# facebookresearch/ReAgent

Measured on NVIDIA H100. Metric: minibatch_td_updates_per_sec_b4096, higher is better.
Workload: dtype f32

## Files before the change

### reagent_b200/csrc/rb200_dqn_tc.cu

```cuda
#include <string.h>

#include <type_traits>

#include "rb200_dqn_tc_layout.cuh"
#include "rb200_wgmma.cuh"

namespace rb200 {

constexpr int kQR = 32;
constexpr int kQSub = 2;
constexpr int kQStages = 3;
constexpr int kQStageBytes = kQSub * (kQKC / 4) * kQFullLbo;
constexpr int kQLboB = 64 * 16 + 16;
constexpr int kQLoOff = 32 * 4;
constexpr int kQEpiThreads = 256;
constexpr int kQThreads = kQEpiThreads + 32;
constexpr int kQMaxTiles = 4;
constexpr int kQMaxSteps = 4 * kMaxLayers;
constexpr int kQMaxSmem = 232448;
static_assert(kQKC == 32, "a chunk is four K = 8 MMA steps");

enum { kStepHidden = 0, kStepLast = 1, kStepBwd = 2 };

struct QStep {
  uint32_t pack_off;
  int16_t N, K;
  int8_t layer, kind, net, in_buf, load_x, save, qdst, out_buf;
};

struct QDev {
  rb200_dqn_args_t a;
  rb200_net_ws_t ws;
  const unsigned char* pack;
  int nsteps, last_fwd_step;
  int buf_off[3];
  int q_off, ldq, lin_off, bar_off;
  int need_zero;
  QStep steps[kQMaxSteps];
};

struct PackJob {
  const float* W;
  int N, K;
  int ld;
  int transpose;
  uint32_t pack_off;
  int chunk0;
};
struct PackDev {
  PackJob jobs[3 * kMaxLayers];
  int njobs;
  unsigned char* pack;
};

constexpr int kPackParts = 4;

__global__ void __launch_bounds__(256) dqn_tc_pack_kernel(const PackDev p) {
  const int chunk = (int)blockIdx.x / kPackParts, part = (int)blockIdx.x % kPackParts;
  int j = 0;
  while (j + 1 < p.njobs && chunk >= p.jobs[j + 1].chunk0) ++j;
  const PackJob job = p.jobs[j];
  const int local = chunk - job.chunk0;
  const int kch = ceil_div(job.K, kQKC);
  const int t = local / kch, c = local - t * kch;
  const ChunkGeo g = chunk_geo(job.N, job.K, t, c);
  const int rows8 = (int)(g.lbo - 16) / 16, kl8 = g.ksteps * 8;
  float* img = reinterpret_cast<float*>(p.pack + job.pack_off + g.off);
  const int m0 = 128 * t, k0 = kQKC * c;
  const int total = rows8 * kl8;
  constexpr int U = 4;
  for (int base = (part * 256 + (int)threadIdx.x); base < total; base += kPackParts * 256 * U) {
    float v[U];
    int o[U];
#pragma unroll
    for (int u = 0; u < U; ++u) {
      const int idx = base + u * kPackParts * 256;
      int m, kk;
      if (job.transpose) { kk = idx / rows8; m = idx - kk * rows8; }
      else { m = idx / kl8; kk = idx - m * kl8; }
      v[u] = 0.f;
      o[u] = -1;
      if (idx < total) {
        o[u] = (kk >> 2) * (int)(g.lbo / 4) + m * 4 + (kk & 3);
        if (m0 + m < job.N && k0 + kk < job.K)
          v[u] = job.transpose ? __ldg(job.W + (size_t)(k0 + kk) * job.ld + m0 + m)
                               : __ldg(job.W + (size_t)(m0 + m) * job.ld + k0 + kk);
      }
    }
#pragma unroll
    for (int u = 0; u < U; ++u)
      if (o[u] >= 0) img[o[u]] = v[u];
  }
}

__device__ __noinline__ float act_fwd_slow(float x, int act) { return act_fwd(x, act); }
__device__ __noinline__ float act_bwd_slow(float y, int act) { return act_bwd_from_out(y, act); }

constexpr int kQCK = kQKC / 8;

template <int NK>
__device__ __forceinline__ void chunk_mma(float (&acc)[32], const uint32_t (&ah)[kQCK][4],
                                          const uint32_t (&al)[kQCK][4], uint32_t b0) {
  wgmma_fence();
#pragma unroll
  for (int kk = 0; kk < NK; ++kk) {
    const uint64_t bd = wgmma_desc(b0 + (uint32_t)(2 * kk) * kQLboB, kQLboB, 128);
    wgmma_rs_n64(acc, ah[kk], bd, 1u);
    wgmma_rs_n32(acc, al[kk], bd, 1u);
  }
  wgmma_commit();
}
template <int NK, typename F>
__device__ __forceinline__ void with_ksteps(int nk, F&& f) {
  if (nk == NK) f(std::integral_constant<int, NK>());
  else if constexpr (NK > 1) with_ksteps<NK - 1>(nk, f);
}

template <bool kWeighted>
__global__ void __launch_bounds__(kQThreads, 1)
dqn_td_tc_kernel(const Mlp q, const Mlp qt, const QDev p) {
  extern __shared__ __align__(128) unsigned char smem_raw[];
  const int tid = threadIdx.x, warp = tid >> 5, lane = tid & 31;
  const rb200_dqn_args_t& a = p.a;
  const int B = a.batch;
  const int row0 = blockIdx.x * kQR;
  const int L = q.n_layers;
  const int A = q.dims[L];

  if (p.need_zero) {
    unsigned nbytes;
    asm("mov.u32 %0, %%dynamic_smem_size;" : "=r"(nbytes));
    for (unsigned i = (unsigned)p.buf_off[0] + tid * 16u; i + 15u < nbytes; i += kQThreads * 16u)
      *reinterpret_cast<float4*>(smem_raw + i) = make_float4(0.f, 0.f, 0.f, 0.f);
  }
  __syncthreads();

  unsigned char* ring = smem_raw;
  float* qarr = reinterpret_cast<float*>(smem_raw + p.q_off);
  float* act_s = reinterpret_cast<float*>(smem_raw + p.lin_off);
  float* mask_s = act_s + kQR * A;
  float* scal_s = mask_s + kQR * A;
  uint64_t* full = reinterpret_cast<uint64_t*>(smem_raw + p.bar_off);
  uint64_t* sfree = full + kQStages;
  const int ldq = p.ldq;

  if (tid == 0) {
    for (int s = 0; s < kQStages; ++s) { mbar_init(full + s, 1); mbar_init(sfree + s, kQEpiThreads / 32); }
    asm volatile("fence.mbarrier_init.release.cluster;\n" ::: "memory");
  }
  __syncthreads();

  const int role = __shfl_sync(0xffffffffu, warp, 0);
  if (role == kQEpiThreads / 32) {
    const bool leader = elect_one();
    int stage = 0;
    uint32_t par = 1;
    for (int s = 0; s < p.nsteps; ++s) {
      const QStep st = p.steps[s];
      const int mt = ceil_div(st.N, 128), kch = ceil_div(st.K, kQKC);
      const uint32_t tile_stride = (uint32_t)(round_up8(st.K) / 4) * kQFullLbo;
      for (int t = 0; t < mt; ++t) {
        const int rows = st.N - 128 * t;
        const uint32_t lbo = (uint32_t)(round_up8(rows < 128 ? rows : 128) * 16 + 16);
        const uint32_t full_bytes = (kQKC / 4) * lbo;
        const int klast = st.K - kQKC * (kch - 1);
        const uint32_t last_bytes = (uint32_t)(round_up8(klast) / 4) * lbo;
        const unsigned char* src = p.pack + st.pack_off + (size_t)t * tile_stride;
        for (int c = 0; c < kch; c += kQSub) {
          const int nsub = kch - c < kQSub ? kch - c : kQSub;
          const uint32_t bytes = (uint32_t)(nsub - 1) * full_bytes + ((c + nsub == kch) ? last_bytes : full_bytes);
          mbar_wait(sfree + stage, par);
          if (leader) {
            mbar_expect_tx(full + stage, bytes);
            bulk_g2s(ring + stage * kQStageBytes, src, bytes, full + stage);
          }
          src += bytes;
          if (++stage == kQStages) { stage = 0; par ^= 1u; }
        }
      }
    }
  } else {
    const int wg = warp >> 2, w4 = warp & 3, g = lane >> 2, tq = lane & 3;
    int ss = 0;
    uint32_t spar = 0;

    constexpr int kXQ = 4;
    const int xS = q.dims[0];
    const int xnq = round_up8(xS) / 4;
    const bool x_in_regs = kQR * xnq <= kXQ * kQEpiThreads;
    float4 xr[kXQ];
    auto x_fetch_one = [&](const float* src, int idx) {
      const bool vec = ((xS & 3) == 0) && ((reinterpret_cast<uintptr_t>(src) & 15) == 0);
      const int r = idx / xnq, qd = idx - r * xnq;
      const int k = 4 * qd, row = row0 + r;
      float4 v = make_float4(0.f, 0.f, 0.f, 0.f);
      if (idx < kQR * xnq && row < B) {
        const float* sp = src + (size_t)row * xS;
        if (vec && k + 3 < xS) {
          asm volatile("ld.global.nc.v4.f32 {%0,%1,%2,%3}, [%4];\n"
                       : "=f"(v.x), "=f"(v.y), "=f"(v.z), "=f"(v.w)
                       : "l"(sp + k));
        } else {
          if (k < xS) v.x = sp[k];
          if (k + 1 < xS) v.y = sp[k + 1];
          if (k + 2 < xS) v.z = sp[k + 2];
          if (k + 3 < xS) v.w = sp[k + 3];
        }
      }
      return v;
    };
    auto x_store_one = [&](int idx, const float4 v) {
      if (idx >= kQR * xnq) return;
      float* base = reinterpret_cast<float*>(smem_raw + p.buf_off[0]);
      const int r = idx / xnq, qd = idx - r * xnq;
      float4 h, l;
      split4(v, h, l);
      const int o = qd * (kQLboB / 4) + r * 4;
      *reinterpret_cast<float4*>(base + o) = h;
      *reinterpret_cast<float4*>(base + o + kQLoOff) = l;
    };
    auto x_fetch = [&](const float* src) {
      if (!x_in_regs) return;
#pragma unroll
      for (int i = 0; i < kXQ; ++i) xr[i] = x_fetch_one(src, tid + i * kQEpiThreads);
    };
    auto x_store = [&](const float* src) {
      if (x_in_regs) {
#pragma unroll
        for (int i = 0; i < kXQ; ++i) x_store_one(tid + i * kQEpiThreads, xr[i]);
      } else {
        for (int idx = tid; idx < kQR * xnq; idx += kQEpiThreads) x_store_one(idx, x_fetch_one(src, idx));
      }
    };
    auto load_loss_inputs = [&]() {
      const float* mask = a.maxq ? a.possible_next_actions_mask : a.next_action;
      for (int idx = tid; idx < kQR * A; idx += kQEpiThreads) {
        const int r = idx / A;
        const bool in = row0 + r < B;
        const size_t g = (size_t)row0 * A + idx;
        act_s[idx] = in ? a.action[g] : 0.f;
        mask_s[idx] = (in && mask) ? mask[g] : 1.f;
      }
      if (tid < kQR) {
        const int row = row0 + tid;
        const bool in = row < B;
        scal_s[tid * 4 + 0] = in ? a.reward[row] : 0.f;
        scal_s[tid * 4 + 1] = in ? a.not_terminal[row] : 0.f;
        scal_s[tid * 4 + 2] = (in && a.discount_mode == RB200_DISCOUNT_POW) ? a.discount_src[row] : 0.f;
      }
    };
    auto step_tiles = [&](const QStep& st) {
      const Mlp& net = st.net ? qt : q;
      const int l = st.layer, N = st.N;
      const int mt = ceil_div(N, 128), kch = ceil_div(st.K, kQKC);
      float* obase = reinterpret_cast<float*>(smem_raw + p.buf_off[st.out_buf]);
      const uint32_t bbase = smem_u32(smem_raw + p.buf_off[st.in_buf]);
      for (int t = 0; t < mt; ++t) {
        const int rows = N - 128 * t;
        const int rows8 = round_up8(rows < 128 ? rows : 128);
        const uint32_t lbo = (uint32_t)(rows8 * 16 + 16);
        const bool live = 64 * wg < rows;
        const int m0 = 64 * wg + 16 * w4 + g;
        const bool ok0 = live && m0 < rows8, ok1 = live && m0 + 8 < rows8;
        float acc[32];
#pragma unroll
        for (int i = 0; i < 32; ++i) {
          acc[i] = 0.f;
          wgmma_fence_operand(acc[i]);
        }
        static_assert(kQSub == 2, "one fragment buffer per chunk of a ring stage");
        const int kfull = st.K / kQKC;
        const int nk_last = round_up8(st.K - kQKC * kfull) / 8;
        uint32_t ah[2][kQCK][4], al[2][kQCK][4];
        auto fetch = [&](uint32_t (&fh)[kQCK][4], uint32_t (&fl)[kQCK][4], int c, int nk) {
          if (c % 2 == 0) mbar_wait(full + ss, spar);
          float v[kQCK][4];
#pragma unroll
          for (int kk = 0; kk < kQCK; ++kk) {
            v[kk][0] = v[kk][1] = v[kk][2] = v[kk][3] = 0.f;
            const unsigned char* s0 = ring + ss * kQStageBytes + (uint32_t)((c % 2) * (kQKC / 4) + 2 * kk) * lbo + tq * 4;
            const unsigned char* s1 = s0 + lbo;
            if (kk < nk && ok0) { v[kk][0] = *reinterpret_cast<const float*>(s0 + m0 * 16); v[kk][2] = *reinterpret_cast<const float*>(s1 + m0 * 16); }
            if (kk < nk && ok1) { v[kk][1] = *reinterpret_cast<const float*>(s0 + (m0 + 8) * 16); v[kk][3] = *reinterpret_cast<const float*>(s1 + (m0 + 8) * 16); }
          }
          if (c % 2 == 1 || c + 1 == kch) {
            __syncwarp();
            if (lane == 0) mbar_arrive(sfree + ss);
            if (++ss == kQStages) { ss = 0; spar ^= 1u; }
          }
#pragma unroll
          for (int kk = 0; kk < kQCK; ++kk)
#pragma unroll
            for (int e = 0; e < 4; ++e) {
              float h, lo_;
              split1(v[kk][e], h, lo_);
              fh[kk][e] = __float_as_uint(h);
              fl[kk][e] = __float_as_uint(lo_);
              wgmma_fence_operand(fh[kk][e]);
              wgmma_fence_operand(fl[kk][e]);
            }
        };
        auto b_of = [&](int c) { return bbase + (uint32_t)(2 * kQCK * c) * kQLboB; };
        if (kfull > 0) fetch(ah[0], al[0], 0, kQCK);
        for (int c = 0; c < kfull; c += 2) {
          chunk_mma<kQCK>(acc, ah[0], al[0], b_of(c));
          if (c + 1 == kfull) break;
          wgmma_wait<1>();
          fetch(ah[1], al[1], c + 1, kQCK);
          chunk_mma<kQCK>(acc, ah[1], al[1], b_of(c + 1));
          if (c + 2 == kfull) break;
          wgmma_wait<1>();
          fetch(ah[0], al[0], c + 2, kQCK);
        }
        if (kfull < kch) {
          wgmma_wait<0>();
          fetch(ah[0], al[0], kfull, nk_last);
          with_ksteps<kQCK>(nk_last, [&](auto nk_c) {
            chunk_mma<decltype(nk_c)::value>(acc, ah[0], al[0], b_of(kfull));
          });
        }
        wgmma_wait<0>();
#pragma unroll
        for (int i = 0; i < 32; ++i) wgmma_fence_operand(acc[i]);
        if (!live) continue;

#pragma unroll
        for (int hh = 0; hh < 2; ++hh) {
          const int n = 128 * t + m0 + 8 * hh;
          const bool valid = n < N;
          float x[8];
#pragma unroll
          for (int i = 0; i < 4; ++i)
#pragma unroll
            for (int e = 0; e < 2; ++e) x[2 * i + e] = acc[4 * i + 2 * hh + e] + acc[4 * (i + 4) + 2 * hh + e];
          auto rowof = [&](int k) { return 8 * (k >> 1) + 2 * tq + (k & 1); };
          float* ob = obase + (n >> 2) * (kQLboB / 4) + (n & 3);
          bool to_operand, to_global;
          float* gdst = nullptr;
          if (st.kind == kStepBwd) {
            const int hact = q.act[l - 1];
            float hv[8];
            if (st.save) {
              const float* hs = p.ws.hidden[l - 1];
#pragma unroll
              for (int k = 0; k < 8; ++k) {
                const int row = row0 + rowof(k);
                hv[k] = (valid && row < B) ? hs[(size_t)row * N + n] : 0.f;
              }
            } else {
#pragma unroll
              for (int k = 0; k < 8; ++k) hv[k] = valid ? ob[rowof(k) * 4] + ob[rowof(k) * 4 + kQLoOff] : 0.f;
            }
            if (hact == RB200_ACT_RELU) {
#pragma unroll
              for (int k = 0; k < 8; ++k) x[k] = hv[k] > 0.f ? x[k] : 0.f;
            } else if (hact != RB200_ACT_LINEAR) {
#pragma unroll
              for (int k = 0; k < 8; ++k) x[k] = valid ? x[k] * act_bwd_slow(hv[k], hact) : 0.f;
            }
            to_operand = l - 1 >= 1;
            to_global = true;
            gdst = p.ws.dz[l - 1];
          } else {
            const float bias = valid ? __ldg(net.params + net.b_off[l] + n) : 0.f;
            const int act = net.act[l];
            if (act == RB200_ACT_RELU) {
#pragma unroll
              for (int k = 0; k < 8; ++k) x[k] = fmaxf(x[k] + bias, 0.f);
            } else if (act == RB200_ACT_LINEAR) {
#pragma unroll
              for (int k = 0; k < 8; ++k) x[k] += bias;
            } else {
#pragma unroll
              for (int k = 0; k < 8; ++k) x[k] = act_fwd_slow(x[k] + bias, act);
            }
            to_operand = st.kind != kStepLast;
            to_global = st.save != 0 && st.kind != kStepLast;
            gdst = to_global ? p.ws.hidden[l] : nullptr;
          }
          if (!valid) continue;
          if (st.kind == kStepLast) {
            float* qd = qarr + st.qdst * kQR * ldq + n;
#pragma unroll
            for (int k = 0; k < 8; ++k) qd[rowof(k) * ldq] = x[k];
            continue;
          }
          if (to_operand) {
#pragma unroll
            for (int k = 0; k < 8; ++k) {
              float h, lo_;
              split1(row0 + rowof(k) < B ? x[k] : 0.f, h, lo_);
              ob[rowof(k) * 4] = h;
              ob[rowof(k) * 4 + kQLoOff] = lo_;
            }
          }
          if (to_global) {
#pragma unroll
            for (int k = 0; k < 8; ++k) {
              const int row = row0 + rowof(k);
              if (row < B) gdst[(size_t)row * N + n] = x[k];
            }
          }
        }
      }
    };
    auto loss_stage = [&]() {
      const float* qa = qarr;
      const float* qb = qarr + kQR * ldq;
      const float* qc = qarr + 2 * kQR * ldq;
      const int r = tid >> 3, sub = tid & 7;
      const int row = row0 + r;
      const bool in = row < B;
      float best = 0.f, sel = 0.f, qsel = 0.f, bsum = 0.f;
      int bi = 0x7fffffff;
      for (int c = sub; c < A; c += 8) {
        const float pen = -1e9f * (1.f - mask_s[r * A + c]);
        const float vt = qb[r * ldq + c] + pen;
        const float key = a.double_q ? (qa[r * ldq + c] + pen) : vt;
        if (bi == 0x7fffffff || key > best) { best = key; bi = c; sel = vt; }
        const float aw = act_s[r * A + c];
        qsel += qc[r * ldq + c] * aw;
        if (a.reward_boost) bsum += aw * a.reward_boost[c];
      }
#pragma unroll
      for (int o = 1; o < 8; o <<= 1) {
        const float ob = __shfl_xor_sync(0xffffffffu, best, o);
        const float os = __shfl_xor_sync(0xffffffffu, sel, o);
        const int oi = __shfl_xor_sync(0xffffffffu, bi, o);
        qsel += __shfl_xor_sync(0xffffffffu, qsel, o);
        bsum += __shfl_xor_sync(0xffffffffu, bsum, o);
        if (oi != 0x7fffffff && (bi == 0x7fffffff || ob > best || (ob == best && oi < bi))) {
          best = ob; bi = oi; sel = os;
        }
      }
      float le = 0.f, g = 0.f;
      if (in) {
        const float rew = scal_s[r * 4 + 0] + bsum;
        const float disc = (a.discount_mode == RB200_DISCOUNT_POW)
                               ? powf(a.gamma, scal_s[r * 4 + 2]) : a.gamma;
        const float tgt = rew + disc * (sel * scal_s[r * 4 + 1]);
        const float d = qsel - tgt;
        const float invB = 1.f / (float)B;
        if (a.loss_kind == RB200_LOSS_HUBER) {
          const float ad = fabsf(d);
          le = ad < 1.f ? 0.5f * d * d : ad - 0.5f;
          g = (d < -1.f) ? -invB : (d > 1.f ? invB : invB * d);
        } else {
          le = d * d;
          g = 2.f * invB * d;
        }
        if (kWeighted) {
          const float w = a.sample_weight[row];
          le *= w;
          g *= w;
        }
        if (sub == 0) {
          if (a.td_target) a.td_target[row] = tgt;
          if (a.next_action_idx) a.next_action_idx[row] = bi;
          if (a.q_selected) a.q_selected[row] = qsel;
        }
      }
      const int A8 = round_up8(A);
      const int lact = q.act[L - 1];
      float* zb = reinterpret_cast<float*>(smem_raw + p.buf_off[2]) + r * 4;
      for (int c = sub; c < A8; c += 8) {
        float v = 0.f;
        if (in && c < A) {
          v = g * act_s[r * A + c];
          if (lact != RB200_ACT_LINEAR) v *= act_bwd_slow(qc[r * ldq + c], lact);
          if (a.all_action_scores) a.all_action_scores[(size_t)row * A + c] = qc[r * ldq + c];
          if (a.do_backward) p.ws.dz[L - 1][(size_t)row * A + c] = v;
        }
        if (a.do_backward) {
          float h, lo_;
          split1(v, h, lo_);
          float* o = zb + (c >> 2) * (kQLboB / 4) + (c & 3);
          o[0] = h;
          o[kQLoOff] = lo_;
        }
      }
      const float ws = warp_sum(sub == 0 ? le : 0.f);
      if (lane == 0) scal_s[kQR * 4 + warp] = ws;
    };


    auto x_src = [&](int lx) { return lx == 1 ? a.state : a.next_state; };
    auto handover = [&]() {
      fence_proxy_async_smem();
      asm volatile("bar.sync 1, %0;\n" ::"n"(kQEpiThreads) : "memory");
    };
    if (p.steps[0].load_x) { x_fetch(x_src(p.steps[0].load_x)); x_store(x_src(p.steps[0].load_x)); }
    load_loss_inputs();
    handover();
    for (int s = 0; s < p.nsteps; ++s) {
      const QStep st = p.steps[s];
      const int lx = (s + 1 < p.nsteps) ? p.steps[s + 1].load_x : 0;
      if (lx) x_fetch(x_src(lx));
      step_tiles(st);
      handover();
      if (s == p.last_fwd_step) {
        loss_stage();
        handover();
      }
      if (lx) {
        x_store(x_src(lx));
        handover();
      }
    }

    if (tid == 0) {
      float loss_partial = 0.f;
      for (int w = 0; w < kQEpiThreads / 32; ++w) loss_partial += scal_s[kQR * 4 + w];
      finish_serial<1>(a.loss_partials, a.tile_counter, {loss_partial},
                       [&](const float (&tot)[1]) { *a.loss = tot[0] / (float)B; });
    }
  }
}

struct QPlan {
  QDev dev;
  PackDev pack;
  int pack_chunks;
  size_t smem_bytes;
  int64_t pack_bytes;
  bool ok;
};

static QPlan make_plan(const rb200_mlp_t* qn, const rb200_mlp_t* qtn, int double_q, int do_backward) {
  QPlan pl;
  memset(&pl, 0, sizeof(pl));
  pl.ok = false;
  const int L = qn->n_layers;
  if (L < 1 || L > kMaxLayers) return pl;
  for (int l = 1; l <= L; ++l)
    if (qn->dims[l] > 128 * kQMaxTiles || qn->dims[l] > 32000) return pl;
  if (qn->dims[0] > 32000 || qn->dims[L] > 256) return pl;

  uint32_t off = 0;
  uint32_t off_on[kMaxLayers], off_tg[kMaxLayers], off_bw[kMaxLayers];
  int nj = 0, nchunks = 0;
  auto add_job = [&](const rb200_mlp_t* net, int l, int transpose) {
    PackJob& j = pl.pack.jobs[nj++];
    j.W = net->params + net->w_off[l];
    j.ld = net->dims[l];
    j.transpose = transpose;
    j.N = transpose ? net->dims[l] : net->dims[l + 1];
    j.K = transpose ? net->dims[l + 1] : net->dims[l];
    j.pack_off = off;
    j.chunk0 = nchunks;
    nchunks += ceil_div(j.N, 128) * ceil_div(j.K, kQKC);
    const uint32_t o = off;
    off += image_bytes(j.N, j.K);
    return o;
  };
  for (int l = 0; l < L; ++l) off_on[l] = add_job(qn, l, 0);
  if (qtn) for (int l = 0; l < L; ++l) off_tg[l] = add_job(qtn, l, 0);
  else for (int l = 0; l < L; ++l) { off_tg[l] = off; off += image_bytes(qn->dims[l + 1], qn->dims[l]); nj++; }
  if (do_backward) for (int l = 1; l < L; ++l) off_bw[l] = add_job(qn, l, 1);
  pl.pack.njobs = nj;
  pl.pack_chunks = nchunks;
  {
    const TcImages im = tc_images(qn, do_backward);
    pl.pack_bytes = im.total_bytes;
    bool same = im.total_bytes == (int64_t)off + 4096;
    for (int l = 0; l < L; ++l) same = same && im.on_fwd[l] == off_on[l] && im.tg_fwd[l] == off_tg[l];
    if (do_backward) for (int l = 1; l < L; ++l) same = same && im.on_bwd[l] == off_bw[l];
    if (!same) return pl;
  }

  int ns = 0;
  auto add_pass = [&](int net, int load_x, int save, int qdst) {
    for (int l = 0; l < L; ++l) {
      QStep& s = pl.dev.steps[ns++];
      s.pack_off = net ? off_tg[l] : off_on[l];
      s.N = (int16_t)qn->dims[l + 1];
      s.K = (int16_t)qn->dims[l];
      s.layer = (int8_t)l;
      s.kind = (l == L - 1) ? kStepLast : kStepHidden;
      s.net = (int8_t)net;
      s.in_buf = (int8_t)(l & 1);
      s.out_buf = (int8_t)((l + 1) & 1);
      s.load_x = (int8_t)(l == 0 ? load_x : 0);
      s.save = (int8_t)save;
      s.qdst = (int8_t)qdst;
    }
  };
  add_pass(1, 2, 0, 1);
  if (double_q) add_pass(0, 2, 0, 0);
  add_pass(0, 1, do_backward ? 1 : 0, 2);
  pl.dev.last_fwd_step = ns - 1;
  if (do_backward) {
    for (int l = L - 1; l >= 1; --l) {
      QStep& s = pl.dev.steps[ns++];
      s.pack_off = off_bw[l];
      s.N = (int16_t)qn->dims[l];
      s.K = (int16_t)qn->dims[l + 1];
      s.layer = (int8_t)l;
      s.kind = kStepBwd;
      s.net = 0;
      s.in_buf = (int8_t)(l == L - 1 ? 2 : ((l + 1) & 1));
      s.out_buf = (int8_t)(l & 1);
      s.save = (int8_t)(l <= L - 3 ? 1 : 0);
    }
  }
  pl.dev.nsteps = ns;
  pl.dev.need_zero = 0;
  for (int l = 0; l <= L; ++l)
    if (qn->dims[l] % 8 != 0) pl.dev.need_zero = 1;

  int maxd[3] = {8, 8, qn->dims[L]};
  for (int i = 0; i < L; ++i) if (qn->dims[i] > maxd[i & 1]) maxd[i & 1] = qn->dims[i];
  size_t o = (size_t)kQStages * kQStageBytes;
  for (int b = 0; b < 3; ++b) {
    pl.dev.buf_off[b] = (int)o;
    o += (size_t)(round_up8(maxd[b]) / 4) * kQLboB;
  }
  pl.dev.ldq = qn->dims[L] + 1;
  pl.dev.q_off = (int)o;
  o += (size_t)3 * kQR * pl.dev.ldq * sizeof(float);
  o = (o + 15) & ~(size_t)15;
  pl.dev.lin_off = (int)o;
  o += ((size_t)2 * kQR * qn->dims[L] + 4 * kQR + 8) * sizeof(float);
  o = (o + 15) & ~(size_t)15;
  pl.dev.bar_off = (int)o;
  o += 2 * kQStages * sizeof(uint64_t);
  pl.smem_bytes = (o + 15) & ~(size_t)15;
  pl.ok = pl.smem_bytes <= (size_t)kQMaxSmem;
  return pl;
}

}

using namespace rb200;

extern "C" int64_t rb200_dqn_tc_workspace_bytes(const rb200_mlp_t* q_net, int32_t double_q,
                                                int32_t do_backward) {
  if (!q_net || validate_mlp(q_net, "q_network")) return 0;
  const QPlan pl = make_plan(q_net, nullptr, double_q, do_backward);
  return pl.ok ? pl.pack_bytes : 0;
}

extern "C" int rb200_dqn_tc_pack(const rb200_mlp_t* q_net, const rb200_mlp_t* q_target,
                                 int32_t double_q, int32_t do_backward, void* pack_ws,
                                 int64_t pack_ws_bytes, void* stream) {
  if (!q_net || !q_target || !pack_ws) { set_last_error("rb200_dqn_tc_pack: null argument"); return RB200_E_INVALID; }
  if (int rc = validate_mlp(q_net, "q_network")) return rc;
  if (int rc = validate_mlp(q_target, "q_network_target")) return rc;
  if (q_net->n_layers != q_target->n_layers) { set_last_error("q_network / target layer count mismatch"); return RB200_E_INVALID; }
  for (int l = 0; l <= q_net->n_layers; ++l)
    if (q_net->dims[l] != q_target->dims[l]) { set_last_error("q_network / target dims mismatch at %d", l); return RB200_E_INVALID; }
  if ((reinterpret_cast<uintptr_t>(pack_ws) & 127) != 0) { set_last_error("pack workspace must be 128-byte aligned"); return RB200_E_INVALID; }
  QPlan pl = make_plan(q_net, q_target, double_q, do_backward);
  if (!pl.ok) { set_last_error("rb200_dqn_tc_pack: shapes do not fit the wgmma path"); return RB200_E_SMEM; }
  if (pack_ws_bytes < pl.pack_bytes) { set_last_error("pack workspace too small: %lld < %lld", (long long)pack_ws_bytes, (long long)pl.pack_bytes); return RB200_E_INVALID; }
  pl.pack.pack = static_cast<unsigned char*>(pack_ws);
  dqn_tc_pack_kernel<<<pl.pack_chunks * kPackParts, 256, 0, (cudaStream_t)stream>>>(pl.pack);
  return check_cuda(cudaGetLastError(), "dqn_tc_pack_kernel launch");
}

extern "C" int rb200_dqn_td_step_tc(const rb200_mlp_t* q_net, const rb200_mlp_t* q_target,
                                    const rb200_dqn_args_t* args, const rb200_net_ws_t* ws,
                                    void* pack_ws, int64_t pack_ws_bytes, int32_t weights_packed,
                                    void* stream) {
  if (!q_net || !q_target || !args || !ws || !pack_ws) { set_last_error("rb200_dqn_td_step_tc: null argument"); return RB200_E_INVALID; }
  if (!weights_packed) {
    if (int rc = rb200_dqn_tc_pack(q_net, q_target, args->double_q, args->do_backward, pack_ws, pack_ws_bytes, stream)) return rc;
  }
  if (int rc = validate_mlp(q_net, "q_network")) return rc;
  if (int rc = validate_mlp(q_target, "q_network_target")) return rc;
  if (q_net->n_layers != q_target->n_layers) { set_last_error("q_network / target layer count mismatch"); return RB200_E_INVALID; }
  for (int l = 0; l <= q_net->n_layers; ++l)
    if (q_net->dims[l] != q_target->dims[l]) { set_last_error("q_network / target dims mismatch at %d", l); return RB200_E_INVALID; }
  if (args->batch <= 0) { set_last_error("batch must be positive"); return RB200_E_INVALID; }
  if (!args->state || !args->next_state || !args->action || !args->reward || !args->not_terminal ||
      !args->loss_partials || !args->loss || !args->tile_counter) {
    set_last_error("rb200_dqn_td_step_tc: required pointer is null"); return RB200_E_INVALID;
  }
  if (!args->maxq && !args->next_action) { set_last_error("SARSA update needs next_action"); return RB200_E_INVALID; }
  if (args->discount_mode == RB200_DISCOUNT_POW && !args->discount_src) { set_last_error("POW discount needs discount_src"); return RB200_E_INVALID; }
  if (args->do_backward) {
    for (int l = 0; l < q_net->n_layers; ++l)
      if (!ws->dz[l] || (l < q_net->n_layers - 1 && !ws->hidden[l])) { set_last_error("workspace buffer missing for layer %d", l); return RB200_E_INVALID; }
  }
  if ((reinterpret_cast<uintptr_t>(pack_ws) & 127) != 0) { set_last_error("pack workspace must be 128-byte aligned"); return RB200_E_INVALID; }
  QPlan pl = make_plan(q_net, q_target, args->double_q, args->do_backward);
  if (!pl.ok) { set_last_error("rb200_dqn_td_step_tc: shapes do not fit the wgmma path"); return RB200_E_SMEM; }
  if (pack_ws_bytes < pl.pack_bytes) { set_last_error("pack workspace too small: %lld < %lld", (long long)pack_ws_bytes, (long long)pl.pack_bytes); return RB200_E_INVALID; }
  pl.dev.a = *args;
  pl.dev.ws = *ws;
  pl.dev.pack = static_cast<const unsigned char*>(pack_ws);
  cudaStream_t st = (cudaStream_t)stream;
  const bool weighted = args->sample_weight != nullptr;
  if (cudaError_t e = weighted ? opt_in_smem<dqn_td_tc_kernel<true>>(pl.smem_bytes)
                               : opt_in_smem<dqn_td_tc_kernel<false>>(pl.smem_bytes))
    return check_cuda(e, "cudaFuncSetAttribute(dqn_td_tc)");
  static int greatest[64] = {};
  static bool have_greatest[64] = {};
  int dev = 0;
  if (cudaError_t e = cudaGetDevice(&dev)) return check_cuda(e, "cudaGetDevice");
  int prio = 0;
  if (dev >= 0 && dev < 64 && have_greatest[dev]) {
    prio = greatest[dev];
  } else {
    int least = 0;
    if (cudaError_t e = cudaDeviceGetStreamPriorityRange(&least, &prio))
      return check_cuda(e, "cudaDeviceGetStreamPriorityRange");
    if (dev >= 0 && dev < 64) { greatest[dev] = prio; have_greatest[dev] = true; }
  }
  const Mlp q = make_mlp(q_net), qt = make_mlp(q_target);
  cudaLaunchConfig_t cfg = {};
  cfg.gridDim = dim3((unsigned)ceil_div(args->batch, kQR));
  cfg.blockDim = dim3(kQThreads);
  cfg.dynamicSmemBytes = pl.smem_bytes;
  cfg.stream = st;
  cudaLaunchAttribute attr[1];
  attr[0].id = cudaLaunchAttributePriority;
  attr[0].val.priority = prio;
  cfg.attrs = attr;
  cfg.numAttrs = 1;
  const cudaError_t e = weighted ? cudaLaunchKernelEx(&cfg, dqn_td_tc_kernel<true>, q, qt, pl.dev)
                                 : cudaLaunchKernelEx(&cfg, dqn_td_tc_kernel<false>, q, qt, pl.dev);
  return check_cuda(e, "dqn_td_tc_kernel launch");
}
```

### reagent_b200/csrc/rb200_wgmma.cuh

```cuda
#pragma once
#include "rb200_common.cuh"

namespace rb200 {

__device__ __forceinline__ uint32_t smem_u32(const void* p) {
  return static_cast<uint32_t>(__cvta_generic_to_shared(p));
}

__device__ __forceinline__ uint64_t wgmma_desc(uint32_t saddr, uint32_t lbo_bytes, uint32_t sbo_bytes) {
  uint64_t d = 0;
  d |= (uint64_t)((saddr >> 4) & 0x3fff);
  d |= (uint64_t)((lbo_bytes >> 4) & 0x3fff) << 16;
  d |= (uint64_t)((sbo_bytes >> 4) & 0x3fff) << 32;
  return d;
}

__device__ __forceinline__ void wgmma_fence() { asm volatile("wgmma.fence.sync.aligned;\n" ::: "memory"); }
__device__ __forceinline__ void wgmma_commit() { asm volatile("wgmma.commit_group.sync.aligned;\n" ::: "memory"); }
template <int N>
__device__ __forceinline__ void wgmma_wait() {
  asm volatile("wgmma.wait_group.sync.aligned %0;\n" ::"n"(N) : "memory");
}
__device__ __forceinline__ void wgmma_fence_operand(uint32_t& r) { asm volatile("" : "+r"(r)::"memory"); }
__device__ __forceinline__ void wgmma_fence_operand(float& r) { asm volatile("" : "+f"(r)::"memory"); }

__device__ __forceinline__ void mbar_init(uint64_t* bar, uint32_t count) {
  asm volatile("mbarrier.init.shared::cta.b64 [%0], %1;\n" ::"r"(smem_u32(bar)), "r"(count));
}
__device__ __forceinline__ void mbar_wait(uint64_t* bar, uint32_t parity) {
  const uint32_t addr = smem_u32(bar);
  for (long long it = 0;; ++it) {
    uint32_t ok;
    asm volatile(
        "{\n\t"
        ".reg .pred p;\n\t"
        "mbarrier.try_wait.parity.shared::cta.b64 p, [%1], %2;\n\t"
        "selp.u32 %0, 1, 0, p;\n\t"
        "}\n"
        : "=r"(ok)
        : "r"(addr), "r"(parity)
        : "memory");
    if (ok) break;
    if (it > 400000LL) __trap();
  }
}

__device__ __forceinline__ void split4(const float4 v, float4& hi, float4& lo) {
  uint32_t h;
  h = (__float_as_uint(v.x) + 0x1000u) & 0xffffe000u; hi.x = __uint_as_float(h); lo.x = v.x - hi.x;
  h = (__float_as_uint(v.y) + 0x1000u) & 0xffffe000u; hi.y = __uint_as_float(h); lo.y = v.y - hi.y;
  h = (__float_as_uint(v.z) + 0x1000u) & 0xffffe000u; hi.z = __uint_as_float(h); lo.z = v.z - hi.z;
  h = (__float_as_uint(v.w) + 0x1000u) & 0xffffe000u; hi.w = __uint_as_float(h); lo.w = v.w - hi.w;
}
__device__ __forceinline__ void split1(float x, float& hi, float& lo) {
  hi = __uint_as_float((__float_as_uint(x) + 0x1000u) & 0xffffe000u);
  lo = x - hi;
}

__device__ __forceinline__ void mbar_arrive(uint64_t* bar) {
  asm volatile("mbarrier.arrive.shared::cta.b64 _, [%0];\n" ::"r"(smem_u32(bar)) : "memory");
}
__device__ __forceinline__ void mbar_expect_tx(uint64_t* bar, uint32_t bytes) {
  asm volatile("mbarrier.arrive.expect_tx.shared::cta.b64 _, [%0], %1;\n" ::"r"(smem_u32(bar)),
               "r"(bytes)
               : "memory");
}
__device__ __forceinline__ void bulk_g2s(void* smem_dst, const void* gsrc, uint32_t bytes,
                                         uint64_t* bar) {
  asm volatile(
      "cp.async.bulk.shared::cluster.global.mbarrier::complete_tx::bytes [%0], [%1], %2, [%3];\n" ::
          "r"(smem_u32(smem_dst)),
      "l"(gsrc), "r"(bytes), "r"(smem_u32(bar))
      : "memory");
}
__device__ __forceinline__ void fence_proxy_async_smem() {
  asm volatile("fence.proxy.async.shared::cta;\n" ::: "memory");
}
__device__ __forceinline__ bool elect_one() {
  uint32_t pred;
  asm volatile(
      "{\n\t"
      ".reg .pred p;\n\t"
      "elect.sync _|p, 0xffffffff;\n\t"
      "selp.u32 %0, 1, 0, p;\n\t"
      "}\n"
      : "=r"(pred));
  return pred != 0;
}

__device__ __forceinline__ void wgmma_ss_n128(float* d, uint64_t da, uint64_t db, uint32_t accumulate) {
  asm volatile(
      "{\n\t.reg .pred p;\n\tsetp.ne.b32 p, %66, 0;\n\t"
      "wgmma.mma_async.sync.aligned.m64n128k8.f32.tf32.tf32 {%0,%1,%2,%3,%4,%5,%6,%7,%8,%9,%10,%11,%12,%13,%14,%15,%16,%17,%18,%19,%20,%21,%22,%23,%24,%25,%26,%27,%28,%29,%30,%31,%32,%33,%34,%35,%36,%37,%38,%39,%40,%41,%42,%43,%44,%45,%46,%47,%48,%49,%50,%51,%52,%53,%54,%55,%56,%57,%58,%59,%60,%61,%62,%63}, %64, %65, p, 1, 1;\n\t}\n"
      : "+f"(d[0]), "+f"(d[1]), "+f"(d[2]), "+f"(d[3]), "+f"(d[4]), "+f"(d[5]), "+f"(d[6]), "+f"(d[7]), "+f"(d[8]), "+f"(d[9]), "+f"(d[10]), "+f"(d[11]), "+f"(d[12]), "+f"(d[13]), "+f"(d[14]), "+f"(d[15]), "+f"(d[16]), "+f"(d[17]), "+f"(d[18]), "+f"(d[19]), "+f"(d[20]), "+f"(d[21]), "+f"(d[22]), "+f"(d[23]), "+f"(d[24]), "+f"(d[25]), "+f"(d[26]), "+f"(d[27]), "+f"(d[28]), "+f"(d[29]), "+f"(d[30]), "+f"(d[31]), "+f"(d[32]), "+f"(d[33]), "+f"(d[34]), "+f"(d[35]), "+f"(d[36]), "+f"(d[37]), "+f"(d[38]), "+f"(d[39]), "+f"(d[40]), "+f"(d[41]), "+f"(d[42]), "+f"(d[43]), "+f"(d[44]), "+f"(d[45]), "+f"(d[46]), "+f"(d[47]), "+f"(d[48]), "+f"(d[49]), "+f"(d[50]), "+f"(d[51]), "+f"(d[52]), "+f"(d[53]), "+f"(d[54]), "+f"(d[55]), "+f"(d[56]), "+f"(d[57]), "+f"(d[58]), "+f"(d[59]), "+f"(d[60]), "+f"(d[61]), "+f"(d[62]), "+f"(d[63])
      : "l"(da), "l"(db), "r"(accumulate));
}

__device__ __forceinline__ void wgmma_rs_n32(float* d, const uint32_t (&a)[4], uint64_t db, uint32_t accumulate) {
  asm volatile(
      "{\n\t.reg .pred p;\n\tsetp.ne.b32 p, %21, 0;\n\t"
      "wgmma.mma_async.sync.aligned.m64n32k8.f32.tf32.tf32 {%0,%1,%2,%3,%4,%5,%6,%7,%8,%9,%10,%11,%12,%13,%14,%15}, {%16,%17,%18,%19}, %20, p, 1, 1;\n\t}\n"
      : "+f"(d[0]), "+f"(d[1]), "+f"(d[2]), "+f"(d[3]), "+f"(d[4]), "+f"(d[5]), "+f"(d[6]), "+f"(d[7]), "+f"(d[8]), "+f"(d[9]), "+f"(d[10]), "+f"(d[11]), "+f"(d[12]), "+f"(d[13]), "+f"(d[14]), "+f"(d[15])
      : "r"(a[0]), "r"(a[1]), "r"(a[2]), "r"(a[3]), "l"(db), "r"(accumulate));
}

__device__ __forceinline__ void wgmma_rs_n64(float* d, const uint32_t (&a)[4], uint64_t db, uint32_t accumulate) {
  asm volatile(
      "{\n\t.reg .pred p;\n\tsetp.ne.b32 p, %37, 0;\n\t"
      "wgmma.mma_async.sync.aligned.m64n64k8.f32.tf32.tf32 {%0,%1,%2,%3,%4,%5,%6,%7,%8,%9,%10,%11,%12,%13,%14,%15,%16,%17,%18,%19,%20,%21,%22,%23,%24,%25,%26,%27,%28,%29,%30,%31}, {%32,%33,%34,%35}, %36, p, 1, 1;\n\t}\n"
      : "+f"(d[0]), "+f"(d[1]), "+f"(d[2]), "+f"(d[3]), "+f"(d[4]), "+f"(d[5]), "+f"(d[6]), "+f"(d[7]), "+f"(d[8]), "+f"(d[9]), "+f"(d[10]), "+f"(d[11]), "+f"(d[12]), "+f"(d[13]), "+f"(d[14]), "+f"(d[15]), "+f"(d[16]), "+f"(d[17]), "+f"(d[18]), "+f"(d[19]), "+f"(d[20]), "+f"(d[21]), "+f"(d[22]), "+f"(d[23]), "+f"(d[24]), "+f"(d[25]), "+f"(d[26]), "+f"(d[27]), "+f"(d[28]), "+f"(d[29]), "+f"(d[30]), "+f"(d[31])
      : "r"(a[0]), "r"(a[1]), "r"(a[2]), "r"(a[3]), "l"(db), "r"(accumulate));
}

}
```

Before: 10530.

## Prefetch next tile's first weight chunk across tiles and steps with warp-specialized registers

Restructures the per-tile MMA loop so the first weight chunk of the next tile, or of the next step, is fetched from the ring and split into hi/lo fragments while the current tile's wgmmas drain. The epilogue becomes a separate lambda and the bias load is hoisted ahead of the MMAs. The ring changes from 3 stages of 2 chunks to 6 stages of 1 chunk. A full producer warpgroup is added so setmaxnreg can move registers to the MMA warps, and sample weights are staged in shared memory. The cost is more register pressure from the persistent prefetch fragments and extra threads that exit immediately.

```diff
diff --git a/reagent_b200/csrc/rb200_dqn_tc.cu b/reagent_b200/csrc/rb200_dqn_tc.cu
--- a/reagent_b200/csrc/rb200_dqn_tc.cu
+++ b/reagent_b200/csrc/rb200_dqn_tc.cu
@@ -8,19 +8,28 @@
 namespace rb200 {
 
 constexpr int kQR = 32;
-constexpr int kQSub = 2;
-constexpr int kQStages = 3;
+constexpr int kQSub = 1;
+constexpr int kQStages = 6;
 constexpr int kQStageBytes = kQSub * (kQKC / 4) * kQFullLbo;
 constexpr int kQLboB = 64 * 16 + 16;
 constexpr int kQLoOff = 32 * 4;
 constexpr int kQEpiThreads = 256;
-constexpr int kQThreads = kQEpiThreads + 32;
+constexpr int kQThreads = kQEpiThreads + 128;
+constexpr int kQProdRegs = 40;
+constexpr int kQMmaRegs = 232;
+static_assert(128 * kQProdRegs + kQEpiThreads * kQMmaRegs <= 65536, "register file of one SM");
 constexpr int kQMaxTiles = 4;
 constexpr int kQMaxSteps = 4 * kMaxLayers;
 constexpr int kQMaxSmem = 232448;
 static_assert(kQKC == 32, "a chunk is four K = 8 MMA steps");
 
 enum { kStepHidden = 0, kStepLast = 1, kStepBwd = 2 };
+
+struct QTile {
+  uint32_t lbo;
+  bool live, ok0, ok1;
+  int kch, kfull, nk_last;
+};
 
 struct QStep {
   uint32_t pack_off;
@@ -151,7 +160,9 @@
   __syncthreads();
 
   const int role = __shfl_sync(0xffffffffu, warp, 0);
-  if (role == kQEpiThreads / 32) {
+  if (role >= kQEpiThreads / 32) {
+    setmaxnreg_dec<kQProdRegs>();
+    if (role != kQEpiThreads / 32) return;
     const bool leader = elect_one();
     int stage = 0;
     uint32_t par = 1;
@@ -180,6 +191,7 @@
       }
     }
   } else {
+    setmaxnreg_inc<kQMmaRegs>();
     const int wg = warp >> 2, w4 = warp & 3, g = lane >> 2, tq = lane & 3;
     int ss = 0;
     uint32_t spar = 0;
@@ -247,162 +259,197 @@
         scal_s[tid * 4 + 0] = in ? a.reward[row] : 0.f;
         scal_s[tid * 4 + 1] = in ? a.not_terminal[row] : 0.f;
         scal_s[tid * 4 + 2] = (in && a.discount_mode == RB200_DISCOUNT_POW) ? a.discount_src[row] : 0.f;
-      }
-    };
-    auto step_tiles = [&](const QStep& st) {
-      const Mlp& net = st.net ? qt : q;
+        if (kWeighted) scal_s[tid * 4 + 3] = in ? a.sample_weight[row] : 0.f;
+      }
+    };
+    const int m0 = 64 * wg + 16 * w4 + g;
+    auto tile_geo = [&](const QStep& st, int t) {
+      QTile G;
+      const int rows = st.N - 128 * t;
+      const int rows8 = round_up8(rows < 128 ? rows : 128);
+      G.lbo = (uint32_t)(rows8 * 16 + 16);
+      G.live = 64 * wg < rows;
+      G.ok0 = G.live && m0 < rows8;
+      G.ok1 = G.live && m0 + 8 < rows8;
+      G.kch = ceil_div(st.K, kQKC);
+      G.kfull = st.K / kQKC;
+      G.nk_last = round_up8(st.K - kQKC * G.kfull) / 8;
+      return G;
+    };
+    uint32_t pf_h[kQCK][4], pf_l[kQCK][4];
+    uint32_t ah[2][kQCK][4], al[2][kQCK][4];
+    auto fetch = [&](uint32_t (&fh)[kQCK][4], uint32_t (&fl)[kQCK][4], const QTile& G, int c, int nk) {
+      const int sub = c % kQSub;
+      if (sub == 0) mbar_wait(full + ss, spar);
+      float v[kQCK][4];
+#pragma unroll
+      for (int kk = 0; kk < kQCK; ++kk) {
+        v[kk][0] = v[kk][1] = v[kk][2] = v[kk][3] = 0.f;
+        const unsigned char* s0 = ring + ss * kQStageBytes + (uint32_t)(sub * (kQKC / 4) + 2 * kk) * G.lbo + tq * 4;
+        const unsigned char* s1 = s0 + G.lbo;
+        if (kk < nk && G.ok0) { v[kk][0] = *reinterpret_cast<const float*>(s0 + m0 * 16); v[kk][2] = *reinterpret_cast<const float*>(s1 + m0 * 16); }
+        if (kk < nk && G.ok1) { v[kk][1] = *reinterpret_cast<const float*>(s0 + (m0 + 8) * 16); v[kk][3] = *reinterpret_cast<const float*>(s1 + (m0 + 8) * 16); }
+      }
+      if (sub == kQSub - 1 || c + 1 == G.kch) {
+        __syncwarp();
+        if (lane == 0) mbar_arrive(sfree + ss);
+        if (++ss == kQStages) { ss = 0; spar ^= 1u; }
+      }
+#pragma unroll
+      for (int kk = 0; kk < kQCK; ++kk)
+#pragma unroll
+        for (int e = 0; e < 4; ++e) {
+          float h, lo_;
+          split1(v[kk][e], h, lo_);
+          fh[kk][e] = __float_as_uint(h);
+          fl[kk][e] = __float_as_uint(lo_);
+          wgmma_fence_operand(fh[kk][e]);
+          wgmma_fence_operand(fl[kk][e]);
+        }
+    };
+    auto fetch_first = [&](const QStep& st, int t) {
+      const QTile G = tile_geo(st, t);
+      fetch(pf_h, pf_l, G, 0, G.kfull > 0 ? kQCK : G.nk_last);
+    };
+
+    auto epilogue = [&](const float (&acc)[32], const float (&bias)[2], const QStep& st, int t) {
       const int l = st.layer, N = st.N;
-      const int mt = ceil_div(N, 128), kch = ceil_div(st.K, kQKC);
       float* obase = reinterpret_cast<float*>(smem_raw + p.buf_off[st.out_buf]);
+#pragma unroll
+      for (int hh = 0; hh < 2; ++hh) {
+        const int n = 128 * t + m0 + 8 * hh;
+        const bool valid = n < N;
+        float x[8];
+#pragma unroll
+        for (int i = 0; i < 4; ++i)
+#pragma unroll
+          for (int e = 0; e < 2; ++e) x[2 * i + e] = acc[4 * i + 2 * hh + e] + acc[4 * (i + 4) + 2 * hh + e];
+        auto rowof = [&](int k) { return 8 * (k >> 1) + 2 * tq + (k & 1); };
+        float* ob = obase + (n >> 2) * (kQLboB / 4) + (n & 3);
+        bool to_operand, to_global;
+        float* gdst = nullptr;
+        if (st.kind == kStepBwd) {
+          const int hact = q.act[l - 1];
+          float hv[8];
+          if (st.save) {
+            const float* hs = p.ws.hidden[l - 1];
+#pragma unroll
+            for (int k = 0; k < 8; ++k) {
+              const int row = row0 + rowof(k);
+              hv[k] = (valid && row < B) ? hs[(size_t)row * N + n] : 0.f;
+            }
+          } else {
+#pragma unroll
+            for (int k = 0; k < 8; ++k) hv[k] = valid ? ob[rowof(k) * 4] + ob[rowof(k) * 4 + kQLoOff] : 0.f;
+          }
+          if (hact == RB200_ACT_RELU) {
+#pragma unroll
+            for (int k = 0; k < 8; ++k) x[k] = hv[k] > 0.f ? x[k] : 0.f;
+          } else if (hact != RB200_ACT_LINEAR) {
+#pragma unroll
+            for (int k = 0; k < 8; ++k) x[k] = valid ? x[k] * act_bwd_slow(hv[k], hact) : 0.f;
+          }
+          to_operand = l - 1 >= 1;
+          to_global = true;
+          gdst = p.ws.dz[l - 1];
+        } else {
+          const int act = (st.net ? qt : q).act[l];
+          if (act == RB200_ACT_RELU) {
+#pragma unroll
+            for (int k = 0; k < 8; ++k) x[k] = fmaxf(x[k] + bias[hh], 0.f);
+          } else if (act == RB200_ACT_LINEAR) {
+#pragma unroll
+            for (int k = 0; k < 8; ++k) x[k] += bias[hh];
+          } else {
+#pragma unroll
+            for (int k = 0; k < 8; ++k) x[k] = act_fwd_slow(x[k] + bias[hh], act);
+          }
+          to_operand = st.kind != kStepLast;
+          to_global = st.save != 0 && st.kind != kStepLast;
+          gdst = to_global ? p.ws.hidden[l] : nullptr;
+        }
+        if (!valid) continue;
+        if (st.kind == kStepLast) {
+          float* qd = qarr + st.qdst * kQR * ldq + n;
+#pragma unroll
+          for (int k = 0; k < 8; ++k) qd[rowof(k) * ldq] = x[k];
+          continue;
+        }
+        if (to_operand) {
+#pragma unroll
+          for (int k = 0; k < 8; ++k) {
+            float h, lo_;
+            split1(row0 + rowof(k) < B ? x[k] : 0.f, h, lo_);
+            ob[rowof(k) * 4] = h;
+            ob[rowof(k) * 4 + kQLoOff] = lo_;
+          }
+        }
+        if (to_global) {
+#pragma unroll
+          for (int k = 0; k < 8; ++k) {
+            const int row = row0 + rowof(k);
+            if (row < B) gdst[(size_t)row * N + n] = x[k];
+          }
+        }
+      }
+    };
+
+    float acc[32], bias[2] = {0.f, 0.f};
+    auto run_tile = [&](const int s, const QStep& st, const int t, const int mt) {
       const uint32_t bbase = smem_u32(smem_raw + p.buf_off[st.in_buf]);
-      for (int t = 0; t < mt; ++t) {
-        const int rows = N - 128 * t;
-        const int rows8 = round_up8(rows < 128 ? rows : 128);
-        const uint32_t lbo = (uint32_t)(rows8 * 16 + 16);
-        const bool live = 64 * wg < rows;
-        const int m0 = 64 * wg + 16 * w4 + g;
-        const bool ok0 = live && m0 < rows8, ok1 = live && m0 + 8 < rows8;
-        float acc[32];
-#pragma unroll
-        for (int i = 0; i < 32; ++i) {
-          acc[i] = 0.f;
-          wgmma_fence_operand(acc[i]);
-        }
-        static_assert(kQSub == 2, "one fragment buffer per chunk of a ring stage");
-        const int kfull = st.K / kQKC;
-        const int nk_last = round_up8(st.K - kQKC * kfull) / 8;
-        uint32_t ah[2][kQCK][4], al[2][kQCK][4];
-        auto fetch = [&](uint32_t (&fh)[kQCK][4], uint32_t (&fl)[kQCK][4], int c, int nk) {
-          if (c % 2 == 0) mbar_wait(full + ss, spar);
-          float v[kQCK][4];
-#pragma unroll
-          for (int kk = 0; kk < kQCK; ++kk) {
-            v[kk][0] = v[kk][1] = v[kk][2] = v[kk][3] = 0.f;
-            const unsigned char* s0 = ring + ss * kQStageBytes + (uint32_t)((c % 2) * (kQKC / 4) + 2 * kk) * lbo + tq * 4;
-            const unsigned char* s1 = s0 + lbo;
-            if (kk < nk && ok0) { v[kk][0] = *reinterpret_cast<const float*>(s0 + m0 * 16); v[kk][2] = *reinterpret_cast<const float*>(s1 + m0 * 16); }
-            if (kk < nk && ok1) { v[kk][1] = *reinterpret_cast<const float*>(s0 + (m0 + 8) * 16); v[kk][3] = *reinterpret_cast<const float*>(s1 + (m0 + 8) * 16); }
-          }
-          if (c % 2 == 1 || c + 1 == kch) {
-            __syncwarp();
-            if (lane == 0) mbar_arrive(sfree + ss);
-            if (++ss == kQStages) { ss = 0; spar ^= 1u; }
-          }
-#pragma unroll
-          for (int kk = 0; kk < kQCK; ++kk)
-#pragma unroll
-            for (int e = 0; e < 4; ++e) {
-              float h, lo_;
-              split1(v[kk][e], h, lo_);
-              fh[kk][e] = __float_as_uint(h);
-              fl[kk][e] = __float_as_uint(lo_);
-              wgmma_fence_operand(fh[kk][e]);
-              wgmma_fence_operand(fl[kk][e]);
-            }
-        };
-        auto b_of = [&](int c) { return bbase + (uint32_t)(2 * kQCK * c) * kQLboB; };
-        if (kfull > 0) fetch(ah[0], al[0], 0, kQCK);
-        for (int c = 0; c < kfull; c += 2) {
-          chunk_mma<kQCK>(acc, ah[0], al[0], b_of(c));
-          if (c + 1 == kfull) break;
-          wgmma_wait<1>();
-          fetch(ah[1], al[1], c + 1, kQCK);
-          chunk_mma<kQCK>(acc, ah[1], al[1], b_of(c + 1));
-          if (c + 2 == kfull) break;
-          wgmma_wait<1>();
-          fetch(ah[0], al[0], c + 2, kQCK);
-        }
-        if (kfull < kch) {
-          wgmma_wait<0>();
-          fetch(ah[0], al[0], kfull, nk_last);
-          with_ksteps<kQCK>(nk_last, [&](auto nk_c) {
-            chunk_mma<decltype(nk_c)::value>(acc, ah[0], al[0], b_of(kfull));
-          });
-        }
-        wgmma_wait<0>();
-#pragma unroll
-        for (int i = 0; i < 32; ++i) wgmma_fence_operand(acc[i]);
-        if (!live) continue;
-
+      auto b_of = [&](int c) { return bbase + (uint32_t)(2 * kQCK * c) * kQLboB; };
+      const QTile G = tile_geo(st, t);
+      if (st.kind != kStepBwd) {
+        const Mlp& net = st.net ? qt : q;
 #pragma unroll
         for (int hh = 0; hh < 2; ++hh) {
           const int n = 128 * t + m0 + 8 * hh;
-          const bool valid = n < N;
-          float x[8];
-#pragma unroll
-          for (int i = 0; i < 4; ++i)
-#pragma unroll
-            for (int e = 0; e < 2; ++e) x[2 * i + e] = acc[4 * i + 2 * hh + e] + acc[4 * (i + 4) + 2 * hh + e];
-          auto rowof = [&](int k) { return 8 * (k >> 1) + 2 * tq + (k & 1); };
-          float* ob = obase + (n >> 2) * (kQLboB / 4) + (n & 3);
-          bool to_operand, to_global;
-          float* gdst = nullptr;
-          if (st.kind == kStepBwd) {
-            const int hact = q.act[l - 1];
-            float hv[8];
-            if (st.save) {
-              const float* hs = p.ws.hidden[l - 1];
-#pragma unroll
-              for (int k = 0; k < 8; ++k) {
-                const int row = row0 + rowof(k);
-                hv[k] = (valid && row < B) ? hs[(size_t)row * N + n] : 0.f;
-              }
-            } else {
-#pragma unroll
-              for (int k = 0; k < 8; ++k) hv[k] = valid ? ob[rowof(k) * 4] + ob[rowof(k) * 4 + kQLoOff] : 0.f;
-            }
-            if (hact == RB200_ACT_RELU) {
-#pragma unroll
-              for (int k = 0; k < 8; ++k) x[k] = hv[k] > 0.f ? x[k] : 0.f;
-            } else if (hact != RB200_ACT_LINEAR) {
-#pragma unroll
-              for (int k = 0; k < 8; ++k) x[k] = valid ? x[k] * act_bwd_slow(hv[k], hact) : 0.f;
-            }
-            to_operand = l - 1 >= 1;
-            to_global = true;
-            gdst = p.ws.dz[l - 1];
-          } else {
-            const float bias = valid ? __ldg(net.params + net.b_off[l] + n) : 0.f;
-            const int act = net.act[l];
-            if (act == RB200_ACT_RELU) {
-#pragma unroll
-              for (int k = 0; k < 8; ++k) x[k] = fmaxf(x[k] + bias, 0.f);
-            } else if (act == RB200_ACT_LINEAR) {
-#pragma unroll
-              for (int k = 0; k < 8; ++k) x[k] += bias;
-            } else {
-#pragma unroll
-              for (int k = 0; k < 8; ++k) x[k] = act_fwd_slow(x[k] + bias, act);
-            }
-            to_operand = st.kind != kStepLast;
-            to_global = st.save != 0 && st.kind != kStepLast;
-            gdst = to_global ? p.ws.hidden[l] : nullptr;
-          }
-          if (!valid) continue;
-          if (st.kind == kStepLast) {
-            float* qd = qarr + st.qdst * kQR * ldq + n;
-#pragma unroll
-            for (int k = 0; k < 8; ++k) qd[rowof(k) * ldq] = x[k];
-            continue;
-          }
-          if (to_operand) {
-#pragma unroll
-            for (int k = 0; k < 8; ++k) {
-              float h, lo_;
-              split1(row0 + rowof(k) < B ? x[k] : 0.f, h, lo_);
-              ob[rowof(k) * 4] = h;
-              ob[rowof(k) * 4 + kQLoOff] = lo_;
-            }
-          }
-          if (to_global) {
-#pragma unroll
-            for (int k = 0; k < 8; ++k) {
-              const int row = row0 + rowof(k);
-              if (row < B) gdst[(size_t)row * N + n] = x[k];
-            }
-          }
-        }
-      }
+          bias[hh] = (G.live && n < st.N) ? __ldg(net.params + net.b_off[st.layer] + n) : 0.f;
+        }
+      }
+#pragma unroll
+      for (int i = 0; i < 32; ++i) {
+        acc[i] = 0.f;
+        wgmma_fence_operand(acc[i]);
+      }
+      if (G.kfull > 0) {
+        chunk_mma<kQCK>(acc, pf_h, pf_l, b_of(0));
+      } else {
+        with_ksteps<kQCK>(G.nk_last, [&](auto nk_c) {
+          chunk_mma<decltype(nk_c)::value>(acc, pf_h, pf_l, b_of(0));
+        });
+      }
+      for (int c = 1; c < G.kfull; c += 2) {
+        if (c > 1) wgmma_wait<1>();
+        fetch(ah[1], al[1], G, c, kQCK);
+        chunk_mma<kQCK>(acc, ah[1], al[1], b_of(c));
+        if (c + 1 == G.kfull) break;
+        wgmma_wait<1>();
+        fetch(ah[0], al[0], G, c + 1, kQCK);
+        chunk_mma<kQCK>(acc, ah[0], al[0], b_of(c + 1));
+      }
+      if (G.kfull > 0 && G.kfull < G.kch) {
+        wgmma_wait<0>();
+        fetch(ah[0], al[0], G, G.kfull, G.nk_last);
+        with_ksteps<kQCK>(G.nk_last, [&](auto nk_c) {
+          chunk_mma<decltype(nk_c)::value>(acc, ah[0], al[0], b_of(G.kfull));
+        });
+      }
+      if (t + 1 < mt || s + 1 < p.nsteps) {
+        if (G.kch > 1) wgmma_wait<1>();
+        else wgmma_wait<0>();
+        if (t + 1 < mt) fetch_first(st, t + 1);
+        else fetch_first(p.steps[s + 1], 0);
+      }
+      wgmma_wait<0>();
+#pragma unroll
+      for (int i = 0; i < 32; ++i) wgmma_fence_operand(acc[i]);
+      if (G.live) epilogue(acc, bias, st, t);
+    };
+    auto step_tiles = [&](int s) {
+      const QStep st = p.steps[s];
+      const int mt = ceil_div(st.N, 128);
+      for (int t = 0; t < mt; ++t) run_tile(s, st, t, mt);
     };
     auto loss_stage = [&]() {
       const float* qa = qarr;
@@ -450,7 +497,7 @@
           g = 2.f * invB * d;
         }
         if (kWeighted) {
-          const float w = a.sample_weight[row];
+          const float w = scal_s[r * 4 + 3];
           le *= w;
           g *= w;
         }
@@ -491,12 +538,12 @@
     };
     if (p.steps[0].load_x) { x_fetch(x_src(p.steps[0].load_x)); x_store(x_src(p.steps[0].load_x)); }
     load_loss_inputs();
+    fetch_first(p.steps[0], 0);
     handover();
     for (int s = 0; s < p.nsteps; ++s) {
-      const QStep st = p.steps[s];
       const int lx = (s + 1 < p.nsteps) ? p.steps[s + 1].load_x : 0;
       if (lx) x_fetch(x_src(lx));
-      step_tiles(st);
+      step_tiles(s);
       handover();
       if (s == p.last_fwd_step) {
         loss_stage();
diff --git a/reagent_b200/csrc/rb200_wgmma.cuh b/reagent_b200/csrc/rb200_wgmma.cuh
--- a/reagent_b200/csrc/rb200_wgmma.cuh
+++ b/reagent_b200/csrc/rb200_wgmma.cuh
@@ -24,9 +24,19 @@
 __device__ __forceinline__ void wgmma_fence_operand(uint32_t& r) { asm volatile("" : "+r"(r)::"memory"); }
 __device__ __forceinline__ void wgmma_fence_operand(float& r) { asm volatile("" : "+f"(r)::"memory"); }
 
+template <int N>
+__device__ __forceinline__ void setmaxnreg_dec() {
+  asm volatile("setmaxnreg.dec.sync.aligned.u32 %0;\n" ::"n"(N));
+}
+template <int N>
+__device__ __forceinline__ void setmaxnreg_inc() {
+  asm volatile("setmaxnreg.inc.sync.aligned.u32 %0;\n" ::"n"(N));
+}
+
 __device__ __forceinline__ void mbar_init(uint64_t* bar, uint32_t count) {
   asm volatile("mbarrier.init.shared::cta.b64 [%0], %1;\n" ::"r"(smem_u32(bar)), "r"(count));
 }
+static __device__ __noinline__ void mbar_timeout() { __trap(); }
 __device__ __forceinline__ void mbar_wait(uint64_t* bar, uint32_t parity) {
   const uint32_t addr = smem_u32(bar);
   for (long long it = 0;; ++it) {
@@ -41,7 +51,7 @@
         : "r"(addr), "r"(parity)
         : "memory");
     if (ok) break;
-    if (it > 400000LL) __trap();
+    if (it > 400000LL) mbar_timeout();
   }
 }
 
```

Measured after the change: 10590 (median of 6 runs). No clear change (+0.6%).
